# qitianwu/SGFormer

Measured on NVIDIA H100. Metric: nodes/sec fwd+bwd, higher is better.
Workload: dtype bf16

## Files before the change

### include/sgformer_b200.h

```cpp
#ifndef SGFORMER_B200_H
#define SGFORMER_B200_H

#include <stddef.h>
#include <stdint.h>

#ifdef __cplusplus
extern "C" {
#endif

#define SGF_F32 0
#define SGF_BF16 1

#define SGF_ERR_ARG (-1)
#define SGF_ERR_UNSUPPORTED (-2)
#define SGF_ERR_DRIVER (-3)

const char* sgf_version(void);
int64_t sgf_launch_count(void);
int sgf_set_device(int device);

int sgf_csr_build_ws_bytes(int64_t nnz, int64_t n, size_t* bytes );
int sgf_csr_build(const int64_t* edge_index , int64_t nnz, int64_t n, int by_source,
                  int self_loop_mode, int64_t* rowptr , int32_t* col, float* dinv ,
                  void* ws, size_t ws_bytes, void* stream);
// ... 94 lines not shown
    int64_t rows; int32_t n_out;
    int32_t epi;
    void* out; int64_t ldo; int32_t out_dtype;
    const float* bias;
    const void* aux; int64_t ld_aux; int32_t aux_dtype;
    const float* row_scale;
    float alpha, beta;
    const float* alpha_dev; const float* beta_dev;
    int32_t relu, accumulate;
    float nf;
    const float* nf_dev;
    float* den_out;
    const float* r1_row; const float* r1_col;
    float* col_sum; float* col_sumsq;
    int32_t schedule;
} sgf_gemm_nt_args;
int sgf_gemm_nt(const sgf_gemm_nt_args* args , void* stream);

#define SGF_TN_MAX_PAIRS 6
typedef struct {
    const void* a; int64_t lda; int32_t m;
    const void* b; int64_t ldb; int32_t n;
    int64_t rows;
    float* out; int64_t ldo; int32_t transpose_out;
    float alpha, beta; const float* alpha_dev;
    void* ws; size_t ws_bytes;
    int32_t n_pairs;
    int32_t a_off[SGF_TN_MAX_PAIRS], b_off[SGF_TN_MAX_PAIRS];
} sgf_gemm_tn_args;
int sgf_gemm_tn_ws_bytes(int32_t m, int32_t n, int64_t rows, size_t* bytes);
int sgf_gemm_tn(const sgf_gemm_tn_args* args , void* stream);

// ... 135 lines not shown
```

### sgformer_b200/_lib.py

```python
import ctypes as C
import os

from . import _build

_i32, _i64, _f32, _u64, _vp, _sz = C.c_int32, C.c_int64, C.c_float, C.c_uint64, C.c_void_p, C.c_size_t
SGF_MAX_SRC, SGF_MAX_SEG = 4, 16
F32, BF16 = 0, 1
EPI_AFFINE, EPI_ATTN_APPLY, EPI_ATTN_GRAM = 0, 1, 2


class GemmNtArgs(C.Structure):
    _fields_ = [
        ("a", _vp * SGF_MAX_SRC), ("lda", _i64 * SGF_MAX_SRC), ("a_cols", _i64 * SGF_MAX_SRC),
        ("b", _vp * SGF_MAX_SRC), ("ldb", _i64 * SGF_MAX_SRC), ("b_cols", _i64 * SGF_MAX_SRC),
        ("n_a", _i32), ("n_b", _i32), ("n_seg", _i32),
        ("seg_a", _i32 * SGF_MAX_SEG), ("seg_akoff", _i32 * SGF_MAX_SEG), ("seg_b", _i32 * SGF_MAX_SEG),
        ("seg_bkoff", _i32 * SGF_MAX_SEG), ("seg_klen", _i32 * SGF_MAX_SEG),
        ("b_tail", _vp), ("ldb_tail", _i64),
        ("rows", _i64), ("n_out", _i32),
        ("epi", _i32),
        ("out", _vp), ("ldo", _i64), ("out_dtype", _i32),
        ("bias", _vp),
        ("aux", _vp), ("ld_aux", _i64), ("aux_dtype", _i32),
        ("row_scale", _vp),
        ("alpha", _f32), ("beta", _f32),
        ("alpha_dev", _vp), ("beta_dev", _vp),
        ("relu", _i32), ("accumulate", _i32),
        ("nf", _f32), ("nf_dev", _vp),
        ("den_out", _vp),
        ("r1_row", _vp), ("r1_col", _vp),
        ("col_sum", _vp), ("col_sumsq", _vp),
        ("schedule", _i32),
    ]


class AttnGramArgs(C.Structure):
    _fields_ = [
        ("h", _i32), ("m", _i32), ("d", _i32), ("n_nodes", _i64),
        ("wq", _vp), ("bq", _vp), ("wk", _vp), ("bk", _vp), ("wv", _vp), ("bv", _vp),
        ("ld_wq", _i64), ("ld_wk", _i64), ("ld_wv", _i64),
        ("G", _vp), ("s", _vp),
        ("kx", _vp), ("qx", _vp), ("vx", _vp), ("z1", _vp), ("q1", _vp), ("v1", _vp), ("S", _vp),
        ("Bt", _vp), ("tail", _vp), ("bt", _vp), ("sc", _vp),
        ("P", _vp), ("pg", _vp), ("cs", _vp), ("sg", _vp),
        ("dwq", _vp), ("dbq", _vp), ("dwk", _vp), ("dbk", _vp), ("dwv", _vp), ("dbv", _vp),
        ("bcat", _vp), ("a4", _vp),
        ("ws", _vp), ("ws_floats", _i64),
# ... 43 lines not shown
    "sgf_remove_self_loops": (C.c_int, [_vp, _i64, _vp, _vp, _vp, _sz, _vp]),
    "sgf_add_self_loops": (C.c_int, [_vp, _i64, _i64, _vp, _vp]),
    "sgf_subgraph": (C.c_int, [_vp, _i64, _i64, _vp, _i64, _vp, _vp, _vp, _vp, _sz, _vp]),
    "sgf_spmm": (C.c_int, [_vp, _vp, _vp, _vp, _i64, _vp, _i64, _i64, C.c_int, C.c_int, _i64, _vp]),
    "sgf_spmm_flagged": (C.c_int, [_vp, _vp, _vp, _vp, _i64, _vp, _i64, _i64, C.c_int, C.c_int, _i64, _vp, _i64, C.c_int, _vp]),
    "sgf_spmm_range": (C.c_int, [_vp, _vp, _vp, _vp, _i64, _vp, _i64, _i64, C.c_int, C.c_int, _vp, _vp, _vp, _vp, _i64, _vp]),
    "sgf_csr_row_splits": (C.c_int, [_vp, _vp, _i64, _vp, C.c_int, _vp, _vp]),
    "sgf_signal": (C.c_int, [_vp, C.c_uint32, _vp]),
    "sgf_set_dropout_epoch": (C.c_int, [_vp]),
    "sgf_advance_dropout_epoch": (C.c_int, [_vp, _vp]),
    "sgf_memcpy_async": (C.c_int, [_vp, _vp, _sz, _vp]),
    "sgf_wait_flags": (C.c_int, [_vp, C.c_int, _vp]),
    "sgf_csr_build_rot": (C.c_int, [_vp, _i64, _i64, _i64, _i64, C.c_int, C.c_int, _i64, _i64, _vp, _vp, _vp, _vp, _sz, _vp]),
    "sgf_spmm_heavy": (C.c_int, [_vp, _vp, _vp, _i64, _vp, _i64, C.c_int, C.c_int, _vp, _vp, _i64, _vp, _vp, _vp, _i64, _vp]),
    "sgf_gemm_nt": (C.c_int, [C.POINTER(GemmNtArgs), _vp]),
    "sgf_gemm_tn_ws_bytes": (C.c_int, [_i32, _i32, _i64, C.POINTER(_sz)]),
    "sgf_gemm_tn": (C.c_int, [C.POINTER(GemmTnArgs), _vp]),
    "sgf_reduce_ws_bytes": (C.c_int, [_i32, C.POINTER(_sz)]),
    "sgf_colstats": (C.c_int, [_vp, _i64, _i64, C.c_int, C.c_int, _vp, _vp, _vp, _vp, _sz, _vp]),
    "sgf_ln_fwd": (C.c_int, [_vp, _vp, _i64, _i64, C.c_int, C.c_int, _f32, _f32, _vp, _vp, C.c_int, C.c_int, _f32,
                             _u64, _vp, _vp, _vp]),
    "sgf_ln_bwd": (C.c_int, [_vp, _vp, _vp, _i64, _i64, C.c_int, C.c_int, _f32, _f32, _vp, _vp, _vp, C.c_int, C.c_int,
                             _f32, _u64, _f32, _vp, _vp, _vp, _vp, _vp, _sz, _vp]),
    "sgf_ln_bwd_attn": (C.c_int, [_vp, _vp, _vp, _vp, _i64, _i64, C.c_int, C.c_int, _f32, _f32, _vp, _vp, _vp, C.c_int, C.c_int,
                                  _f32, _u64, _f32, _vp, _vp, _vp, _vp, _vp, _vp, _vp, _vp, _vp, _vp, _sz, _vp]),
    "sgf_ln_fwd_graph": (C.c_int, [_vp, _vp, _vp, _i64, _i64, C.c_int, C.c_int, _f32, _f32, _f32, _vp, _vp, C.c_int, C.c_int,
                                   _f32, _u64, _vp, _vp, _vp]),
    "sgf_ln_bwd_attn_graph": (C.c_int, [_vp, _vp, _vp, _vp, _vp, _i64, _i64, C.c_int, C.c_int, _f32, _f32, _f32, _vp, _vp, _vp,
                                        C.c_int, _f32, _u64, _f32, _vp, _vp, _vp, _vp, _vp, _vp, _vp, _vp, _vp, _vp, _vp, _vp,
                                        _sz, _vp]),
# ... 89 lines not shown
```

### sgformer_b200/csrc/gemm_tc.cu

```cuda
#include "common.cuh"
#include "launch_count.h"
#include "../../include/sgformer_b200.h"

#include <cstdlib>
#include <cstring>
#include <mutex>

namespace sgf {

typedef CUresult (*PFN_encodeTiled)(CUtensorMap*, CUtensorMapDataType, cuuint32_t, void*, const cuuint64_t*, const cuuint64_t*,
                                    const cuuint32_t*, const cuuint32_t*, CUtensorMapInterleave, CUtensorMapSwizzle,
                                    CUtensorMapL2promotion, CUtensorMapFloatOOBfill);
static PFN_encodeTiled get_encode() {
    static PFN_encodeTiled fn = nullptr;
    static std::once_flag once;
    std::call_once(once, [] {
        void* p = nullptr;
        cudaDriverEntryPointQueryResult q;
        if (cudaGetDriverEntryPoint("cuTensorMapEncodeTiled", &p, cudaEnableDefault, &q) == cudaSuccess &&
            q == cudaDriverEntryPointSuccess)
            fn = (PFN_encodeTiled)p;
    });
    return fn;
}
// ... 14 lines not shown
    return r == CUDA_SUCCESS ? SGF_OK : SGF_ERR_DRIVER;
}
static int make_tmap_bf16(CUtensorMap* tm, const void* base, int64_t rows, int64_t cols, int64_t ld, int box_rows) {
    return make_tmap_2d(tm, base, 1, rows, cols, ld, box_rows);
}

namespace nt {
constexpr int BM = 128, BK = 64, STAGES = 3;
constexpr int MMA_WARPS = 8;
constexpr int THREADS = 32 * (MMA_WARPS + 4);
constexpr int A_BYTES = BM * BK * 2;
constexpr int B_BYTES_MAX = (256 + 16) * BK * 2;
constexpr int STAGE_BYTES = A_BYTES + B_BYTES_MAX;
constexpr int WSTG_BYTES = 16 * 128;
constexpr int BAR_BYTES = 512;
constexpr int STAT_COLS = 1024;
constexpr int STAT_BYTES = 2 * STAT_COLS * 4;
constexpr int SMEM_BYTES = STAGES * STAGE_BYTES + MMA_WARPS * 2 * WSTG_BYTES + BAR_BYTES + STAT_BYTES + 1024;
constexpr int RES_BYTES = (256 + 16) * 256 * 2;
constexpr int RES_MAX_KB = 16;
constexpr int RES_MIN_STAGES = 3, RING_MAX = 8;
constexpr int SMEM_LIMIT = 232448;
constexpr int RES_FIXED_BYTES = MMA_WARPS * WSTG_BYTES + BAR_BYTES + STAT_BYTES + 1024;
constexpr int SMEM_BYTES_RES = RES_BYTES + RES_MIN_STAGES * A_BYTES + RES_FIXED_BYTES;
static_assert(SMEM_BYTES <= SMEM_LIMIT && SMEM_BYTES_RES <= SMEM_LIMIT, "exceeds the 227 KB of dynamic shared memory per CTA");

struct Seg {
    int a_idx, a_koff, b_idx, b_koff, k_blocks;
};
struct Params {
    int64_t rows;
    int n_out, bn_main, bn_pad, has_tail, n_blocks;
    int64_t num_tiles;
    int b_res;
    int res_bytes, ring_stages;
    int64_t chunk;
    int n_seg, total_kb;
    Seg seg[SGF_MAX_SEG];
    int epi;
    void* out; int64_t ldo; int out_dtype;
    const float* bias;
    const void* aux; int64_t ld_aux; int aux_dtype;
    const float* row_scale;
    float alpha, beta;
    const float* alpha_dev; const float* beta_dev;
    int relu, accumulate;
    float nf; const float* nf_dev; float* den_out;
    const float* r1_row; const float* r1_col;
    int tma_store;
    float* col_sum; float* col_sumsq;
};
struct Tmaps {
    CUtensorMap a[SGF_MAX_SRC];
    CUtensorMap b[SGF_MAX_SRC];
    CUtensorMap tail;
    CUtensorMap out;
};

__device__ __forceinline__ float load1(const void* base, int dtype, int64_t off) {
    return dtype == 1 ? __bfloat162float(static_cast<const __nv_bfloat16*>(base)[off]) : static_cast<const float*>(base)[off];
}
__device__ __forceinline__ void store1(void* base, int dtype, int64_t off, float v) {
    if (dtype == 1) static_cast<__nv_bfloat16*>(base)[off] = __float2bfloat16_rn(v);
    else static_cast<float*>(base)[off] = v;
}
// ... 34 lines not shown
                    c0 += p.chunk;
                    if (c0 >= cnt) return false;
                }
                i = c0;
            }
        }
        const int64_t cend = c0 + p.chunk < cnt ? c0 + p.chunk : cnt;
        m_blk = (int)(blockIdx.x + i * gridDim.x);
        n_blk = nb;
        first = i == c0;
        last = i == cend - 1;
        return true;
    }
};

enum : int { F_BIAS = 1, F_AUX = 2, F_RELU = 4, F_ROWSCALE = 8, F_ACCUM = 16, F_R1 = 32, F_ATTN = 64, F_GENERIC = 128 };

template <bool GEN>
__device__ __forceinline__ void load_piece(const void* src, int dtype, int64_t ld, const int64_t* rows, const bool* row_ok,
                                           int col0, int n_out, bool nc, float* d) {
#pragma unroll
    for (int c = 0; c < 4; ++c)
#pragma unroll
        for (int s = 0; s < 2; ++s) {
            const int col = col0 + 8 * c;
            const int64_t off = rows[s] * ld + col;
            float a0 = 0.f, a1 = 0.f;
            if (!GEN) {
                if (row_ok[s]) {
                    const uint32_t* q = reinterpret_cast<const uint32_t*>(static_cast<const __nv_bfloat16*>(src) + off);
                    unpack_bf16x2(nc ? __ldg(q) : *q, a0, a1);
// ... 2 lines not shown
                if (row_ok[s] && col < n_out) a0 = load1(src, dtype, off);
                if (row_ok[s] && col + 1 < n_out) a1 = load1(src, dtype, off + 1);
            }
            d[4 * c + 2 * s] = a0;
            d[4 * c + 2 * s + 1] = a1;
        }
}

template <int F>
__global__ void __launch_bounds__(THREADS, 1) gemm_nt_kernel(const __grid_constant__ Tmaps tm, const __grid_constant__ Params p) {
    extern __shared__ uint8_t smem_raw[];
    uint8_t* smem = reinterpret_cast<uint8_t*>((reinterpret_cast<uintptr_t>(smem_raw) + 1023) & ~static_cast<uintptr_t>(1023));
    const bool res = p.b_res != 0;
    uint8_t* bres = smem;
    uint8_t* ring = res ? smem + p.res_bytes : smem;
    const int ring_stages = res ? p.ring_stages : STAGES;
    const int ring_stride = res ? A_BYTES : STAGE_BYTES;
    const int stg_per_warp = res ? 1 : 2;
    uint8_t* staging = ring + ring_stages * ring_stride;
    uint64_t* full = reinterpret_cast<uint64_t*>(staging + MMA_WARPS * stg_per_warp * WSTG_BYTES);
    uint64_t* empty = full + RING_MAX;
    uint64_t* bres_full = empty + RING_MAX;
    uint64_t* bres_empty = bres_full + RES_MAX_KB;
    float* stat_sm = reinterpret_cast<float*>(reinterpret_cast<uint8_t*>(full) + BAR_BYTES);
    static_assert((2 * RING_MAX + 2 * RES_MAX_KB) * 8 <= BAR_BYTES, "barrier area");
    static_assert(STAGES <= RING_MAX, "ring barriers");
    const bool want_stats = p.col_sum != nullptr || p.col_sumsq != nullptr;

    const int warp = threadIdx.x >> 5;
    const int lane = threadIdx.x & 31;
    const uint32_t b_tx = p.bn_pad * BK * 2 + (p.has_tail ? 16 * BK * 2 : 0);
    if (want_stats)
        for (int i = threadIdx.x; i < 2 * STAT_COLS; i += THREADS) stat_sm[i] = 0.f;

    if (threadIdx.x == 0) {
        for (int i = 0; i < p.n_seg; ++i) {
            tma_prefetch_desc(&tm.a[p.seg[i].a_idx]);
            tma_prefetch_desc(&tm.b[p.seg[i].b_idx]);
        }
        if (p.has_tail) tma_prefetch_desc(&tm.tail);
        if (p.tma_store) tma_prefetch_desc(&tm.out);
        for (int s = 0; s < ring_stages; ++s) { mbar_init(&full[s], 1); mbar_init(&empty[s], MMA_WARPS); }
        for (int s = 0; s < RES_MAX_KB; ++s) { mbar_init(&bres_full[s], 1); mbar_init(&bres_empty[s], MMA_WARPS); }
        fence_barrier_init();
    }
    __syncthreads();

    if (warp >= MMA_WARPS) {
// ... 31 lines not shown
            }
        }
        return;
    }
    consumer_regs();

    constexpr bool GEN = (F & F_GENERIC) != 0;
    const bool f_bias = GEN ? p.bias != nullptr : (F & F_BIAS) != 0;
    const bool f_aux = GEN ? p.aux != nullptr : (F & F_AUX) != 0;
    const bool f_relu = GEN ? p.relu != 0 : (F & F_RELU) != 0;
    const bool f_rs = GEN ? p.row_scale != nullptr : (F & F_ROWSCALE) != 0;
    const bool f_acc = GEN ? p.accumulate != 0 : (F & F_ACCUM) != 0;
    const bool f_r1 = GEN ? p.r1_row != nullptr : (F & F_R1) != 0;
    const bool f_attn = GEN ? (p.epi == SGF_EPI_ATTN_APPLY || p.epi == SGF_EPI_ATTN_GRAM) : (F & F_ATTN) != 0;
    const bool f_tma = GEN ? p.tma_store != 0 : true;
    const bool f_stats = GEN ? want_stats : false;
    const int out_dtype = GEN ? p.out_dtype : 1;
    const int wg = warp >> 2;
    const int wq = warp & 3;
    const int rr = lane >> 2;
    const int cq = 2 * (lane & 3);
    float alpha = p.alpha, beta = p.beta;
    if (p.alpha_dev) alpha *= *p.alpha_dev;
    if (p.beta_dev) beta *= *p.beta_dev;
    const float nfv = (f_attn && p.nf_dev) ? *p.nf_dev : p.nf;
    const int GW = out_dtype == 1 ? 64 : 32;
    const int ppg = GW / 32;
    const int n_pieces = (p.bn_main + 31) / 32;
    const int nch = p.bn_pad / 64;
    uint8_t* wstg = staging + warp * stg_per_warp * WSTG_BYTES;
    const uint32_t a_off = wg * 64 * BK * 2;

    float acc[4][32];
    float acct[8];
    uint32_t gcount = 0;
    int stage = 0; uint32_t phase = 0;
    TileIter ti(p);
    while (ti.next()) {
        const int m_blk = ti.m_blk, n_blk = ti.n_blk;
        const int64_t row_w = (int64_t)m_blk * BM + wg * 64 + wq * 16;
        const int col_base = n_blk * p.bn_main;
        if (!GEN && (f_acc || f_aux) && lane < 16 && row_w + lane < p.rows) {
            if (f_acc) bulk_prefetch_l2(static_cast<const __nv_bfloat16*>(p.out) + (row_w + lane) * p.ldo + col_base, p.bn_main * 2);
            if (f_aux) bulk_prefetch_l2(static_cast<const __nv_bfloat16*>(p.aux) + (row_w + lane) * p.ld_aux + col_base, p.bn_main * 2);
        }
        int prev = 0;
        for (int kbg = 0; kbg < p.total_kb; ++kbg) {
            if (res && ti.first) mbar_wait(&bres_full[kbg], (uint32_t)(ti.group & 1));
            mbar_wait(&full[stage], phase);
            const uint32_t sa = smem_u32(ring + stage * ring_stride) + a_off;
            const uint32_t sb = res ? smem_u32(bres) + (uint32_t)kbg * b_tx : smem_u32(ring + stage * ring_stride) + A_BYTES;
            wgmma_fence();
#pragma unroll
            for (int k = 0; k < BK / 16; ++k) {
                const uint64_t da = make_smem_desc_sw128(sa + k * 32, 16, 1024);
                const uint32_t sc = (kbg > 0 || k > 0) ? 1u : 0u;
#pragma unroll
                for (int j = 0; j < 4; ++j)
                    if (j < nch) wgmma_n64<0, 0>(acc[j], da, make_smem_desc_sw128(sb + j * 8192 + k * 32, 16, 1024), sc);
                if (p.has_tail) wgmma_n16<0, 0>(acct, da, make_smem_desc_sw128(sb + p.bn_pad * BK * 2 + k * 32, 16, 1024), sc);
            }
            wgmma_commit();
            if (res) wgmma_wait<1>();
            else wgmma_wait<0>();
            __syncwarp();
            if (lane == 0 && (kbg > 0 || !res)) {
                mbar_arrive(&empty[res ? prev : stage]);
                if (res && ti.last) mbar_arrive(&bres_empty[kbg - 1]);
            }
            prev = stage;
            if (++stage == ring_stages) { stage = 0; phase ^= 1; }
        }
        wgmma_wait<0>();
#pragma unroll
        for (int j = 0; j < 4; ++j) fence_regs(acc[j]);
        fence_regs(acct);
        __syncwarp();
        if (lane == 0 && res) {
            mbar_arrive(&empty[prev]);
            if (ti.last) mbar_arrive(&bres_empty[p.total_kb - 1]);
        }

        const int64_t rows[2] = {row_w + rr, row_w + rr + 8};
        const bool row_ok[2] = {rows[0] < p.rows, rows[1] < p.rows};
        float rs[2] = {1.f, 1.f}, r1r[2] = {0.f, 0.f}, inv_den[2] = {1.f, 1.f};
#pragma unroll
        for (int s = 0; s < 2; ++s) {
            if (f_rs && row_ok[s]) rs[s] = p.row_scale[rows[s]];
            if (f_r1 && row_ok[s]) r1r[s] = p.r1_row[rows[s]];
        }
        if (f_attn) {
#pragma unroll
            for (int s = 0; s < 2; ++s) {
                const float den = __shfl_sync(0xffffffffu, acct[2 * s], lane & ~3) + nfv;
                inv_den[s] = 1.f / den;
                if (row_ok[s] && p.den_out && n_blk == 0 && (lane & 3) == 0) p.den_out[rows[s]] = den;
// ... 9 lines not shown
                    if (stg_per_warp == 2) bulk_wait_read<1>(); else bulk_wait_read<0>();
                }
                __syncwarp();
            }
            float v[16];
#pragma unroll
            for (int i = 0; i < 16; ++i) v[i] = acc[pc >> 1][(pc & 1) * 16 + i];
            const int col0 = col_base + pc * 32 + cq;
            float ax[16], old[16];
            if (f_aux) load_piece<GEN>(p.aux, p.aux_dtype, p.ld_aux, rows, row_ok, col0, p.n_out, true, ax);
            if (f_acc) load_piece<GEN>(p.out, out_dtype, p.ldo, rows, row_ok, col0, p.n_out, false, old);
#pragma unroll
            for (int i = 0; i < 16; ++i) {
                const int s = (i >> 1) & 1;
                const int col = col0 + 8 * (i >> 2) + (i & 1);
                const bool cok = !GEN || col < p.n_out;
                float x = v[i];
                if (f_attn) {
                    if (f_aux) x += nfv * ax[i];
                    if (f_bias && cok) x += __ldg(p.bias + col);
                    x *= inv_den[s];
                } else {
                    x *= alpha;
                    if (f_aux) x += beta * ax[i];
                    if (f_bias && cok) x += __ldg(p.bias + col);
                    if (f_r1 && cok) x += r1r[s] * __ldg(p.r1_col + col);
                    if (f_relu) x = fmaxf(x, 0.f);
                    if (f_rs) x *= rs[s];
                }
                if (f_acc) x += old[i];
                v[i] = x;
// ... 12 lines not shown
                            const int chunk = (2 * c + (cq >> 2)) ^ (r & 7);
                            *reinterpret_cast<float2*>(tile + r * 128 + chunk * 16 + 4 * (cq & 3)) = make_float2(v[4 * c + 2 * s], v[4 * c + 2 * s + 1]);
                        }
                    }
            } else if constexpr (GEN) {
#pragma unroll
                for (int i = 0; i < 16; ++i) {
                    const int s = (i >> 1) & 1;
                    const int col = col0 + 8 * (i >> 2) + (i & 1);
                    if (row_ok[s] && col < p.n_out) store1(p.out, out_dtype, rows[s] * p.ldo + col, v[i]);
                }
            }
            if (f_tma && (pp == ppg - 1 || pc == n_pieces - 1)) {
                fence_proxy_async_smem();
                __syncwarp();
                if (lane == 0) {
                    tma_store_2d(&tm.out, wstg + buf * WSTG_BYTES, col_base + g * GW, (int32_t)row_w);
                    bulk_commit();
                }
                if (f_stats) {
                    const uint8_t* tile = wstg + buf * WSTG_BYTES;
                    const int64_t valid_rows = p.rows - row_w;
                    for (int cg = lane; cg < GW; cg += 32) {
                        const int colg = col_base + g * GW + cg;
                        if (colg >= p.n_out || colg >= col_base + p.bn_main) continue;
                        float s1 = 0.f, s2 = 0.f;
                        for (int r = 0; r < 16 && r < valid_rows; ++r) {
                            float x;
                            if (out_dtype == 1) {
                                const int chunk = (cg >> 3) ^ (r & 7);
                                x = __bfloat162float(*reinterpret_cast<const __nv_bfloat16*>(tile + r * 128 + chunk * 16 + (cg & 7) * 2));
                            } else {
                                const int chunk = (cg >> 2) ^ (r & 7);
                                x = *reinterpret_cast<const float*>(tile + r * 128 + chunk * 16 + (cg & 3) * 4);
                            }
                            s1 += x;
                            s2 += x * x;
                        }
                        atomicAdd(&stat_sm[colg], s1);
                        atomicAdd(&stat_sm[STAT_COLS + colg], s2);
                    }
                }
                ++gcount;
            }
        }
    }
    if (f_tma && lane == 0) bulk_wait<0>();
    if (f_stats) {
        named_bar_sync(3, 32 * MMA_WARPS);
        for (int i = threadIdx.x; i < p.n_out; i += 32 * MMA_WARPS) {
            if (p.col_sum) atomicAdd(&p.col_sum[i], stat_sm[i]);
            if (p.col_sumsq) atomicAdd(&p.col_sumsq[i], stat_sm[STAT_COLS + i]);
        }
    }
}
}

constexpr int FLUSH_KB = 16;
#ifndef SGF_TN_DIAG
#define SGF_TN_DIAG 0
#endif

__device__ __forceinline__ void red_add_f32(float* p, float v) {
    asm volatile("red.global.add.f32 [%0], %1;" :: "l"(p), "f"(v) : "memory");
}
__device__ __forceinline__ void flush_acc_red(float (&acc)[4][32], float* ws, int mp, int mrow, int cq, int j0, int ncols, bool add) {
#pragma unroll
    for (int j = 0; j < 4; ++j) {
// ... 303 lines not shown
        } else {
            i = t - h * h;
            c = un;
        }
        float acc = 0.f;
        for (int part = 0; part < nparts; ++part) acc += ws[((int64_t)part * (un + 1) + c) * mp + i];
        if (t < h * h) G[(int64_t)(t / h) * ldg + t % h] = acc;
        else s[i] = acc;
    }
}
}
}

using namespace sgf;

extern "C" int sgf_gemm_nt(const sgf_gemm_nt_args* a, void* stream) {
    if (!a || a->rows < 0 || a->n_out <= 0 || a->n_seg <= 0 || a->n_seg > SGF_MAX_SEG || a->n_a <= 0 || a->n_a > SGF_MAX_SRC ||
        a->n_b <= 0 || a->n_b > SGF_MAX_SRC || !a->out)
        return SGF_ERR_ARG;
    if (a->out_dtype != 0 && a->out_dtype != 1) return SGF_ERR_ARG;
    if (a->aux && a->aux_dtype != 0 && a->aux_dtype != 1) return SGF_ERR_ARG;
    if (a->rows == 0) return SGF_OK;
    const bool has_tail = a->b_tail != nullptr;
    if (has_tail && (a->n_b != 1 || a->n_out > 256)) return SGF_ERR_ARG;
    if (a->epi == SGF_EPI_ATTN_APPLY && (!has_tail || !a->aux)) return SGF_ERR_ARG;
    if (a->epi == SGF_EPI_ATTN_GRAM && (!has_tail || !a->bias || !a->nf_dev || a->aux)) return SGF_ERR_ARG;
    if (a->epi != SGF_EPI_AFFINE && a->epi != SGF_EPI_ATTN_APPLY && a->epi != SGF_EPI_ATTN_GRAM) return SGF_ERR_ARG;
    if ((a->r1_row == nullptr) != (a->r1_col == nullptr)) return SGF_ERR_ARG;

    nt::Params p;
// ... 47 lines not shown
    if (has_tail && (rc = make_tmap_bf16(&tm.tail, a->b_tail, 16, a->b_cols[0], a->ldb_tail, 16))) return rc;

    p.epi = a->epi;
    p.out = a->out; p.ldo = a->ldo; p.out_dtype = a->out_dtype;
    p.bias = a->bias;
    p.aux = a->aux; p.ld_aux = a->ld_aux; p.aux_dtype = a->aux_dtype;
    p.row_scale = a->row_scale;
    p.alpha = a->alpha; p.beta = a->beta; p.alpha_dev = a->alpha_dev; p.beta_dev = a->beta_dev;
    p.relu = a->relu; p.accumulate = a->accumulate;
    p.nf = a->nf; p.nf_dev = a->nf_dev; p.den_out = a->den_out;
    p.r1_row = a->r1_row; p.r1_col = a->r1_col;
    {
        const int es = a->out_dtype == 1 ? 2 : 4;
        p.tma_store = ((reinterpret_cast<uintptr_t>(a->out) & 15) == 0 && (a->ldo * es) % 16 == 0) ? 1 : 0;
        if (p.tma_store && (rc = make_tmap_2d(&tm.out, a->out, a->out_dtype, a->rows, a->n_out, a->ldo, 16))) return rc;
        p.col_sum = a->col_sum; p.col_sumsq = a->col_sumsq;
        if ((p.col_sum || p.col_sumsq) && (!p.tma_store || a->n_out > nt::STAT_COLS)) return SGF_ERR_UNSUPPORTED;
    }

    {
        const int64_t b_tx = (int64_t)(p.bn_pad + (has_tail ? 16 : 0)) * nt::BK * 2;
        const bool fits = p.total_kb <= nt::RES_MAX_KB && b_tx * p.total_kb <= nt::RES_BYTES;
        if (a->schedule == SGF_GEMM_RESIDENT_B && !fits) return SGF_ERR_UNSUPPORTED;
        p.b_res = (fits && (a->schedule == SGF_GEMM_RESIDENT_B || (a->schedule == SGF_GEMM_AUTO && p.n_blocks == 1))) ? 1 : 0;
        p.chunk = p.n_blocks == 1 ? (int64_t)1 << 40 : 4;
        p.res_bytes = (int)(b_tx * p.total_kb);
        const int st = (nt::SMEM_LIMIT - p.res_bytes - nt::RES_FIXED_BYTES) / nt::A_BYTES;
        p.ring_stages = st < nt::RING_MAX ? st : nt::RING_MAX;
        if (p.b_res && p.ring_stages < nt::RES_MIN_STAGES) return SGF_ERR_UNSUPPORTED;
    }
    const int64_t work = p.b_res ? m_blocks : p.num_tiles;
    const int64_t grid = work < num_sms() ? work : num_sms();
    const int smem_bytes = p.b_res ? p.res_bytes + p.ring_stages * nt::A_BYTES + nt::RES_FIXED_BYTES : nt::SMEM_BYTES;

    int feat = (a->bias ? nt::F_BIAS : 0) | (a->aux ? nt::F_AUX : 0) | (a->relu ? nt::F_RELU : 0) |
               (a->row_scale ? nt::F_ROWSCALE : 0) | (a->accumulate ? nt::F_ACCUM : 0) | (a->r1_row ? nt::F_R1 : 0) |
               (a->epi != SGF_EPI_AFFINE ? nt::F_ATTN : 0);
    const bool al16 = (!a->bias || (reinterpret_cast<uintptr_t>(a->bias) & 15) == 0) &&
                      (!a->r1_col || (reinterpret_cast<uintptr_t>(a->r1_col) & 15) == 0) &&
                      (!a->aux || (a->aux_dtype == 1 && (reinterpret_cast<uintptr_t>(a->aux) & 15) == 0 && (a->ld_aux * 2) % 16 == 0));
    const bool fast_ok = p.tma_store && a->out_dtype == 1 && a->n_out % 32 == 0 && al16 && !p.col_sum && !p.col_sumsq &&
                         p.n_blocks * p.bn_main == a->n_out;
    static const bool no_special = [] { const char* e = getenv("SGF_GEMM_NT_GENERIC"); return e && e[0] == '1'; }();
    if (!fast_ok || no_special) feat = nt::F_GENERIC;
    const int smem_max = nt::SMEM_LIMIT;
#define SGF_NT_CASE(FEAT)                                                                                                   \
    case (FEAT): {                                                                                                         \
        static bool attr_set = false;                                                                                      \
        if (!attr_set) {                                                                                                   \
            SGF_CUDA_TRY(cudaFuncSetAttribute(nt::gemm_nt_kernel<(FEAT)>, cudaFuncAttributeMaxDynamicSharedMemorySize,     \
                                              smem_max));                                                                  \
            attr_set = true;                                                                                               \
        }                                                                                                                  \
        nt::gemm_nt_kernel<(FEAT)><<<(unsigned)grid, nt::THREADS, smem_bytes, (cudaStream_t)stream>>>(tm, p);              \
        launched = true;                                                                                                   \
    } break;
    for (int attempt = 0; attempt < 2; ++attempt) {
        bool launched = false;
        switch (feat) {
            SGF_NT_CASE(0)
            SGF_NT_CASE(nt::F_BIAS)
            SGF_NT_CASE(nt::F_BIAS | nt::F_RELU)
            SGF_NT_CASE(nt::F_ROWSCALE)
            SGF_NT_CASE(nt::F_ACCUM)
            SGF_NT_CASE(nt::F_AUX)
            SGF_NT_CASE(nt::F_AUX | nt::F_ACCUM)
            SGF_NT_CASE(nt::F_AUX | nt::F_BIAS)
            SGF_NT_CASE(nt::F_AUX | nt::F_R1)
            SGF_NT_CASE(nt::F_AUX | nt::F_ATTN)
            SGF_NT_CASE(nt::F_BIAS | nt::F_ATTN)
            SGF_NT_CASE(nt::F_BIAS | nt::F_R1)
            SGF_NT_CASE(nt::F_BIAS | nt::F_R1 | nt::F_ACCUM)
            SGF_NT_CASE(nt::F_GENERIC)
            default: break;
        }
        if (launched) break;
        feat = nt::F_GENERIC;
    }
#undef SGF_NT_CASE
    SGF_LAUNCH_CHECK(); count_launch();
    return SGF_OK;
}

static inline int tn_splits(int64_t kb_total, int m_blocks) {
    const int64_t cap = num_sms() / m_blocks > 0 ? num_sms() / m_blocks : 1;
    return (int)(kb_total < cap ? (kb_total < 1 ? 1 : kb_total) : cap);
}

extern "C" int sgf_gemm_tn_ws_bytes(int32_t m, int32_t n, int64_t rows, size_t* bytes) {
    if (!bytes || m <= 0 || m > 256 || n <= 0 || n > 256 || rows < 0) return SGF_ERR_ARG;
    const int m_blocks = (m + 127) / 128, un = (n + 15) / 16 * 16;
// ... 126 lines not shown
```

### sgformer_b200/kernels.py

```python
from __future__ import annotations

import ctypes as C
import os
import threading
from dataclasses import dataclass
from typing import Optional, Sequence, Tuple

import torch

from . import _lib
from ._lib import BF16, EPI_AFFINE, EPI_ATTN_APPLY, EPI_ATTN_GRAM, F32, AttnGramArgs, GemmNtArgs, GemmTnArgs, check

Tensor = torch.Tensor
_tls = threading.local()


def lib():
    return _lib.load()


def _use(t: Tensor):
    if not t.is_cuda:
        raise RuntimeError("sgformer_b200 kernels need CUDA tensors (no CPU fallback); got device " + str(t.device))
    idx = t.device.index if t.device.index is not None else torch.cuda.current_device()
# ... 588 lines not shown
        raise ValueError(f"out is {tuple(out.shape)}, expected ({rows}, {n_out})")
    args.out, args.ldo, args.out_dtype = out.data_ptr(), ldo, dcode(out)
    args.bias = _p(_f32vec(bias, n_out, "bias"))
    if aux is not None:
        ar, ac, lda_ = _mat(aux, "aux")
        if ar != rows or ac != n_out:
            raise ValueError("aux shape mismatch")
        args.aux, args.ld_aux, args.aux_dtype = aux.data_ptr(), lda_, dcode(aux)
    args.row_scale = _p(_f32vec(row_scale, rows, "row_scale"))
    args.alpha, args.beta = alpha, beta
    args.alpha_dev, args.beta_dev = _p(alpha_dev), _p(beta_dev)
    args.relu, args.accumulate = int(relu), int(accumulate)
    args.nf, args.den_out = nf, _p(_f32vec(den_out, rows, "den_out"))
    args.nf_dev = _p(_f32vec(nf_dev, 1, "nf_dev"))
    args.r1_row, args.r1_col = _p(_f32vec(r1_row, rows, "r1_row")), _p(_f32vec(r1_col, n_out, "r1_col"))
    fused_stats = (col_sum is not None or col_sumsq is not None) and stats_fusable(out)
    if fused_stats:
        args.col_sum, args.col_sumsq = _p(_f32vec(col_sum, n_out, "col_sum")), _p(_f32vec(col_sumsq, n_out, "col_sumsq"))
    args.schedule = GEMM_NT_SCHEDULE if schedule is None else schedule
    check(lib().sgf_gemm_nt(C.byref(args), _stream()), "sgf_gemm_nt")
    if (col_sum is not None or col_sumsq is not None) and not fused_stats:
        s_, q_ = colstats(out, want_sum=col_sum is not None, want_sumsq=col_sumsq is not None)
        if col_sum is not None:
            col_sum.add_(s_)
        if col_sumsq is not None:
            col_sumsq.add_(q_)
    return out


GEMM_NT_SCHEDULE = int(os.environ.get("SGF_GEMM_NT_SCHEDULE", "0"))

FUSE_GEMM_STATS = os.environ.get("SGF_FUSED_STATS", "0") == "1"


def stats_fusable(out: Tensor) -> bool:
    return FUSE_GEMM_STATS and out.data_ptr() % 16 == 0 and (out.stride(0) * out.element_size()) % 16 == 0 and \
        out.shape[1] <= 1024


def _tn_once(a: Tensor, lda: int, m: int, b: Tensor, ldb: int, n: int, rows: int, out: Tensor, transpose_out: bool,
             alpha: float, beta: float, alpha_dev: Optional[Tensor], pairs: Sequence[Tuple[int, int]] = ()):
    nbytes = C.c_size_t(0)
    check(lib().sgf_gemm_tn_ws_bytes(m, n, rows, C.byref(nbytes)), "sgf_gemm_tn_ws_bytes")
    ws = torch.empty(max(nbytes.value, 4), dtype=torch.uint8, device=out.device)
    args = GemmTnArgs()
    args.a, args.lda, args.m = a.data_ptr(), lda, m
    args.b, args.ldb, args.n = b.data_ptr(), ldb, n
    args.rows = rows
    args.out, args.ldo, args.transpose_out = out.data_ptr(), out.stride(0), int(transpose_out)
    args.alpha, args.beta, args.alpha_dev = alpha, beta, _p(alpha_dev)
    args.ws, args.ws_bytes = ws.data_ptr(), nbytes.value
    args.n_pairs = len(pairs)
# ... 537 lines not shown
```

Baseline: 12.65 million.

## Add specialized fused column-stats and f32-output paths to NT GEMM with dynamic ring stages

Column sum and sum-of-squares now accumulate in registers per warp and are reduced once per CTA into a global partial buffer, with the last CTA (found via an atomic counter) doing the final cross-CTA reduction. This replaces the old shared-memory atomics in the generic path, which also frees the fixed stats shared-memory region. A specialized f32-output template is added, and the streaming ring's stage count is now sized from the actual B tile size, so smaller tiles get deeper pipelines. Fused stats remain off by default behind SGF_FUSED_STATS and need a workspace allocation plus a memset per call.

New measurement: 12.70 million (median of 6 runs). No clear change (+0.4%).

```diff
diff --git a/include/sgformer_b200.h b/include/sgformer_b200.h
--- a/include/sgformer_b200.h
+++ b/include/sgformer_b200.h
@@ -132,8 +132,10 @@
     const float* r1_row; const float* r1_col;
     float* col_sum; float* col_sumsq;
     int32_t schedule;
+    void* stat_ws; size_t stat_ws_bytes;
 } sgf_gemm_nt_args;
 int sgf_gemm_nt(const sgf_gemm_nt_args* args , void* stream);
+int sgf_gemm_nt_stats_ws_bytes(int32_t n_out, size_t* bytes);
 
 #define SGF_TN_MAX_PAIRS 6
 typedef struct {
diff --git a/sgformer_b200/_lib.py b/sgformer_b200/_lib.py
--- a/sgformer_b200/_lib.py
+++ b/sgformer_b200/_lib.py
@@ -5,6 +5,7 @@
 
 _i32, _i64, _f32, _u64, _vp, _sz = C.c_int32, C.c_int64, C.c_float, C.c_uint64, C.c_void_p, C.c_size_t
 SGF_MAX_SRC, SGF_MAX_SEG = 4, 16
+SGF_ERR_UNSUPPORTED = -2
 F32, BF16 = 0, 1
 EPI_AFFINE, EPI_ATTN_APPLY, EPI_ATTN_GRAM = 0, 1, 2
 
@@ -31,6 +32,7 @@
         ("r1_row", _vp), ("r1_col", _vp),
         ("col_sum", _vp), ("col_sumsq", _vp),
         ("schedule", _i32),
+        ("stat_ws", _vp), ("stat_ws_bytes", _sz),
     ]
 
 
@@ -104,6 +106,7 @@
     "sgf_csr_build_rot": (C.c_int, [_vp, _i64, _i64, _i64, _i64, C.c_int, C.c_int, _i64, _i64, _vp, _vp, _vp, _vp, _sz, _vp]),
     "sgf_spmm_heavy": (C.c_int, [_vp, _vp, _vp, _i64, _vp, _i64, C.c_int, C.c_int, _vp, _vp, _i64, _vp, _vp, _vp, _i64, _vp]),
     "sgf_gemm_nt": (C.c_int, [C.POINTER(GemmNtArgs), _vp]),
+    "sgf_gemm_nt_stats_ws_bytes": (C.c_int, [_i32, C.POINTER(_sz)]),
     "sgf_gemm_tn_ws_bytes": (C.c_int, [_i32, _i32, _i64, C.POINTER(_sz)]),
     "sgf_gemm_tn": (C.c_int, [C.POINTER(GemmTnArgs), _vp]),
     "sgf_reduce_ws_bytes": (C.c_int, [_i32, C.POINTER(_sz)]),
diff --git a/sgformer_b200/csrc/gemm_tc.cu b/sgformer_b200/csrc/gemm_tc.cu
--- a/sgformer_b200/csrc/gemm_tc.cu
+++ b/sgformer_b200/csrc/gemm_tc.cu
@@ -52,14 +52,14 @@
 constexpr int STAGE_BYTES = A_BYTES + B_BYTES_MAX;
 constexpr int WSTG_BYTES = 16 * 128;
 constexpr int BAR_BYTES = 512;
-constexpr int STAT_COLS = 1024;
-constexpr int STAT_BYTES = 2 * STAT_COLS * 4;
-constexpr int SMEM_BYTES = STAGES * STAGE_BYTES + MMA_WARPS * 2 * WSTG_BYTES + BAR_BYTES + STAT_BYTES + 1024;
+constexpr int STAT_COLS = 256;
+constexpr int STREAM_FIXED_BYTES = MMA_WARPS * 2 * WSTG_BYTES + BAR_BYTES + 1024;
+constexpr int SMEM_BYTES = STAGES * STAGE_BYTES + STREAM_FIXED_BYTES;
 constexpr int RES_BYTES = (256 + 16) * 256 * 2;
 constexpr int RES_MAX_KB = 16;
 constexpr int RES_MIN_STAGES = 3, RING_MAX = 8;
 constexpr int SMEM_LIMIT = 232448;
-constexpr int RES_FIXED_BYTES = MMA_WARPS * WSTG_BYTES + BAR_BYTES + STAT_BYTES + 1024;
+constexpr int RES_FIXED_BYTES = MMA_WARPS * WSTG_BYTES + BAR_BYTES + 1024;
 constexpr int SMEM_BYTES_RES = RES_BYTES + RES_MIN_STAGES * A_BYTES + RES_FIXED_BYTES;
 static_assert(SMEM_BYTES <= SMEM_LIMIT && SMEM_BYTES_RES <= SMEM_LIMIT, "exceeds the 227 KB of dynamic shared memory per CTA");
 
@@ -72,6 +72,7 @@
     int64_t num_tiles;
     int b_res;
     int res_bytes, ring_stages;
+    int stage_bytes;
     int64_t chunk;
     int n_seg, total_kb;
     Seg seg[SGF_MAX_SEG];
@@ -87,6 +88,7 @@
     const float* r1_row; const float* r1_col;
     int tma_store;
     float* col_sum; float* col_sumsq;
+    float* stat_part; unsigned* stat_cnt;
 };
 struct Tmaps {
     CUtensorMap a[SGF_MAX_SRC];
@@ -151,7 +153,67 @@
     }
 };
 
-enum : int { F_BIAS = 1, F_AUX = 2, F_RELU = 4, F_ROWSCALE = 8, F_ACCUM = 16, F_R1 = 32, F_ATTN = 64, F_GENERIC = 128 };
+enum : int { F_BIAS = 1, F_AUX = 2, F_RELU = 4, F_ROWSCALE = 8, F_ACCUM = 16, F_R1 = 32, F_ATTN = 64, F_GENERIC = 128,
+             F_F32 = 256, F_STATS = 512 };
+
+#ifndef SGF_NT_DIAG
+#define SGF_NT_DIAG 0
+#endif
+
+__device__ __forceinline__ void stats_flush(const Params& p, const float (&s1)[4][2], const float (&s2)[4][2], uint8_t* staging,
+                                            int stg_stride, float* grp_sm, unsigned* last_sm, int warp, int lane) {
+    const int n = p.n_out;
+    float* mine = reinterpret_cast<float*>(staging + warp * stg_stride);
+#pragma unroll
+    for (int g = 0; g < 4; ++g) {
+        const int c = 64 * g + 2 * lane;
+        if (c < n) {
+            *reinterpret_cast<float2*>(mine + c) = make_float2(s1[g][0], s1[g][1]);
+            *reinterpret_cast<float2*>(mine + STAT_COLS + c) = make_float2(s2[g][0], s2[g][1]);
+        }
+    }
+    named_bar_sync(3, 32 * MMA_WARPS);
+    float* part = p.stat_part + (size_t)blockIdx.x * 2 * n;
+    for (int i = threadIdx.x; i < 2 * n; i += 32 * MMA_WARPS) {
+        const int off = i < n ? i : STAT_COLS + i - n;
+        float t = 0.f;
+        for (int w = 0; w < MMA_WARPS; ++w) t += reinterpret_cast<const float*>(staging + w * stg_stride)[off];
+        part[i] = t;
+    }
+    __threadfence();
+    named_bar_sync(3, 32 * MMA_WARPS);
+    if (threadIdx.x == 0) *last_sm = atomicAdd(p.stat_cnt, 1u) == gridDim.x - 1;
+    named_bar_sync(3, 32 * MMA_WARPS);
+    if (!*last_sm) return;
+    __threadfence();
+    const int nv = 2 * n / 4, G = 32 * MMA_WARPS / nv, grp = threadIdx.x / nv, v = threadIdx.x % nv;
+    if (grp < G) {
+        float4 a[4];
+#pragma unroll
+        for (int j = 0; j < 4; ++j) a[j] = make_float4(0.f, 0.f, 0.f, 0.f);
+        unsigned b = grp;
+        for (; b + 3 * G < gridDim.x; b += 4 * G)
+#pragma unroll
+            for (int j = 0; j < 4; ++j) {
+                const float4 x = __ldcg(reinterpret_cast<const float4*>(p.stat_part + (size_t)(b + j * G) * 2 * n) + v);
+                a[j].x += x.x; a[j].y += x.y; a[j].z += x.z; a[j].w += x.w;
+            }
+        for (; b < gridDim.x; b += G) {
+            const float4 x = __ldcg(reinterpret_cast<const float4*>(p.stat_part + (size_t)b * 2 * n) + v);
+            a[0].x += x.x; a[0].y += x.y; a[0].z += x.z; a[0].w += x.w;
+        }
+        reinterpret_cast<float4*>(grp_sm)[grp * nv + v] =
+            make_float4((a[0].x + a[1].x) + (a[2].x + a[3].x), (a[0].y + a[1].y) + (a[2].y + a[3].y),
+                        (a[0].z + a[1].z) + (a[2].z + a[3].z), (a[0].w + a[1].w) + (a[2].w + a[3].w));
+    }
+    named_bar_sync(3, 32 * MMA_WARPS);
+    for (int i = threadIdx.x; i < 2 * n; i += 32 * MMA_WARPS) {
+        float t = 0.f;
+        for (int q = 0; q < G; ++q) t += grp_sm[q * 2 * n + i];
+        float* dst = i < n ? p.col_sum + i : p.col_sumsq + (i - n);
+        if (i < n ? p.col_sum != nullptr : p.col_sumsq != nullptr) *dst += t;
+    }
+}
 
 template <bool GEN>
 __device__ __forceinline__ void load_piece(const void* src, int dtype, int64_t ld, const int64_t* rows, const bool* row_ok,
@@ -184,24 +246,22 @@
     const bool res = p.b_res != 0;
     uint8_t* bres = smem;
     uint8_t* ring = res ? smem + p.res_bytes : smem;
-    const int ring_stages = res ? p.ring_stages : STAGES;
-    const int ring_stride = res ? A_BYTES : STAGE_BYTES;
+    const int ring_stages = p.ring_stages;
+    const int ring_stride = res ? A_BYTES : p.stage_bytes;
     const int stg_per_warp = res ? 1 : 2;
     uint8_t* staging = ring + ring_stages * ring_stride;
     uint64_t* full = reinterpret_cast<uint64_t*>(staging + MMA_WARPS * stg_per_warp * WSTG_BYTES);
     uint64_t* empty = full + RING_MAX;
     uint64_t* bres_full = empty + RING_MAX;
     uint64_t* bres_empty = bres_full + RES_MAX_KB;
-    float* stat_sm = reinterpret_cast<float*>(reinterpret_cast<uint8_t*>(full) + BAR_BYTES);
-    static_assert((2 * RING_MAX + 2 * RES_MAX_KB) * 8 <= BAR_BYTES, "barrier area");
+    unsigned* last_sm = reinterpret_cast<unsigned*>(bres_empty + RES_MAX_KB);
+    float* grp_sm = reinterpret_cast<float*>(ring);
+    static_assert((2 * RING_MAX + 2 * RES_MAX_KB) * 8 + 4 <= BAR_BYTES, "barrier area");
     static_assert(STAGES <= RING_MAX, "ring barriers");
-    const bool want_stats = p.col_sum != nullptr || p.col_sumsq != nullptr;
 
     const int warp = threadIdx.x >> 5;
     const int lane = threadIdx.x & 31;
     const uint32_t b_tx = p.bn_pad * BK * 2 + (p.has_tail ? 16 * BK * 2 : 0);
-    if (want_stats)
-        for (int i = threadIdx.x; i < 2 * STAT_COLS; i += THREADS) stat_sm[i] = 0.f;
 
     if (threadIdx.x == 0) {
         for (int i = 0; i < p.n_seg; ++i) {
@@ -263,8 +323,9 @@
     const bool f_r1 = GEN ? p.r1_row != nullptr : (F & F_R1) != 0;
     const bool f_attn = GEN ? (p.epi == SGF_EPI_ATTN_APPLY || p.epi == SGF_EPI_ATTN_GRAM) : (F & F_ATTN) != 0;
     const bool f_tma = GEN ? p.tma_store != 0 : true;
-    const bool f_stats = GEN ? want_stats : false;
-    const int out_dtype = GEN ? p.out_dtype : 1;
+    constexpr bool f_stats = (F & F_STATS) != 0;
+    constexpr bool RAGGED = GEN || (F & F_F32) != 0;
+    const int out_dtype = GEN ? p.out_dtype : ((F & F_F32) ? 0 : 1);
     const int wg = warp >> 2;
     const int wq = warp & 3;
     const int rr = lane >> 2;
@@ -282,6 +343,9 @@
 
     float acc[4][32];
     float acct[8];
+    float st1[4][2], st2[4][2];
+#pragma unroll
+    for (int g = 0; g < 4; ++g) st1[g][0] = st1[g][1] = st2[g][0] = st2[g][1] = 0.f;
     uint32_t gcount = 0;
     int stage = 0; uint32_t phase = 0;
     TileIter ti(p);
@@ -302,6 +366,7 @@
             wgmma_fence();
 #pragma unroll
             for (int k = 0; k < BK / 16; ++k) {
+                if (SGF_NT_DIAG == 2) break;
                 const uint64_t da = make_smem_desc_sw128(sa + k * 32, 16, 1024);
                 const uint32_t sc = (kbg > 0 || k > 0) ? 1u : 0u;
 #pragma unroll
@@ -329,6 +394,7 @@
             mbar_arrive(&empty[prev]);
             if (ti.last) mbar_arrive(&bres_empty[p.total_kb - 1]);
         }
+        if (SGF_NT_DIAG == 1) continue;
 
         const int64_t rows[2] = {row_w + rr, row_w + rr + 8};
         const bool row_ok[2] = {rows[0] < p.rows, rows[1] < p.rows};
@@ -368,7 +434,7 @@
             for (int i = 0; i < 16; ++i) {
                 const int s = (i >> 1) & 1;
                 const int col = col0 + 8 * (i >> 2) + (i & 1);
-                const bool cok = !GEN || col < p.n_out;
+                const bool cok = !RAGGED || col < p.n_out;
                 float x = v[i];
                 if (f_attn) {
                     if (f_aux) x += nfv * ax[i];
@@ -411,31 +477,22 @@
             if (f_tma && (pp == ppg - 1 || pc == n_pieces - 1)) {
                 fence_proxy_async_smem();
                 __syncwarp();
-                if (lane == 0) {
+                if (lane == 0 && SGF_NT_DIAG != 3) {
                     tma_store_2d(&tm.out, wstg + buf * WSTG_BYTES, col_base + g * GW, (int32_t)row_w);
                     bulk_commit();
                 }
                 if (f_stats) {
                     const uint8_t* tile = wstg + buf * WSTG_BYTES;
                     const int64_t valid_rows = p.rows - row_w;
-                    for (int cg = lane; cg < GW; cg += 32) {
-                        const int colg = col_base + g * GW + cg;
-                        if (colg >= p.n_out || colg >= col_base + p.bn_main) continue;
-                        float s1 = 0.f, s2 = 0.f;
+                    if (g * GW + 2 * lane < p.bn_main) {
                         for (int r = 0; r < 16 && r < valid_rows; ++r) {
-                            float x;
-                            if (out_dtype == 1) {
-                                const int chunk = (cg >> 3) ^ (r & 7);
-                                x = __bfloat162float(*reinterpret_cast<const __nv_bfloat16*>(tile + r * 128 + chunk * 16 + (cg & 7) * 2));
-                            } else {
-                                const int chunk = (cg >> 2) ^ (r & 7);
-                                x = *reinterpret_cast<const float*>(tile + r * 128 + chunk * 16 + (cg & 3) * 4);
-                            }
-                            s1 += x;
-                            s2 += x * x;
+                            float x0, x1;
+                            unpack_bf16x2(*reinterpret_cast<const uint32_t*>(tile + r * 128 + (((lane >> 2) ^ (r & 7)) * 16) + (lane & 3) * 4), x0, x1);
+                            st1[g][0] += x0;
+                            st1[g][1] += x1;
+                            st2[g][0] = fmaf(x0, x0, st2[g][0]);
+                            st2[g][1] = fmaf(x1, x1, st2[g][1]);
                         }
-                        atomicAdd(&stat_sm[colg], s1);
-                        atomicAdd(&stat_sm[STAT_COLS + colg], s2);
                     }
                 }
                 ++gcount;
@@ -443,12 +500,9 @@
         }
     }
     if (f_tma && lane == 0) bulk_wait<0>();
-    if (f_stats) {
-        named_bar_sync(3, 32 * MMA_WARPS);
-        for (int i = threadIdx.x; i < p.n_out; i += 32 * MMA_WARPS) {
-            if (p.col_sum) atomicAdd(&p.col_sum[i], stat_sm[i]);
-            if (p.col_sumsq) atomicAdd(&p.col_sumsq[i], stat_sm[STAT_COLS + i]);
-        }
+    if constexpr (f_stats) {
+        __syncwarp();
+        stats_flush(p, st1, st2, staging, stg_per_warp * WSTG_BYTES, grp_sm, last_sm, warp, lane);
     }
 }
 }
@@ -782,6 +836,12 @@
 
 using namespace sgf;
 
+extern "C" int sgf_gemm_nt_stats_ws_bytes(int32_t n_out, size_t* bytes) {
+    if (!bytes || n_out <= 0) return SGF_ERR_ARG;
+    *bytes = 256 + (size_t)num_sms() * 2 * (size_t)n_out * sizeof(float);
+    return SGF_OK;
+}
+
 extern "C" int sgf_gemm_nt(const sgf_gemm_nt_args* a, void* stream) {
     if (!a || a->rows < 0 || a->n_out <= 0 || a->n_seg <= 0 || a->n_seg > SGF_MAX_SEG || a->n_a <= 0 || a->n_a > SGF_MAX_SRC ||
         a->n_b <= 0 || a->n_b > SGF_MAX_SRC || !a->out)
@@ -859,8 +919,6 @@
         const int es = a->out_dtype == 1 ? 2 : 4;
         p.tma_store = ((reinterpret_cast<uintptr_t>(a->out) & 15) == 0 && (a->ldo * es) % 16 == 0) ? 1 : 0;
         if (p.tma_store && (rc = make_tmap_2d(&tm.out, a->out, a->out_dtype, a->rows, a->n_out, a->ldo, 16))) return rc;
-        p.col_sum = a->col_sum; p.col_sumsq = a->col_sumsq;
-        if ((p.col_sum || p.col_sumsq) && (!p.tma_store || a->n_out > nt::STAT_COLS)) return SGF_ERR_UNSUPPORTED;
     }
 
     {
@@ -873,10 +931,16 @@
         const int st = (nt::SMEM_LIMIT - p.res_bytes - nt::RES_FIXED_BYTES) / nt::A_BYTES;
         p.ring_stages = st < nt::RING_MAX ? st : nt::RING_MAX;
         if (p.b_res && p.ring_stages < nt::RES_MIN_STAGES) return SGF_ERR_UNSUPPORTED;
+        if (!p.b_res) {
+            p.stage_bytes = (int)(nt::A_BYTES + b_tx);
+            const int ss = (nt::SMEM_LIMIT - nt::STREAM_FIXED_BYTES) / p.stage_bytes;
+            p.ring_stages = ss < nt::RING_MAX ? ss : nt::RING_MAX;
+        }
     }
     const int64_t work = p.b_res ? m_blocks : p.num_tiles;
     const int64_t grid = work < num_sms() ? work : num_sms();
-    const int smem_bytes = p.b_res ? p.res_bytes + p.ring_stages * nt::A_BYTES + nt::RES_FIXED_BYTES : nt::SMEM_BYTES;
+    const int smem_bytes = p.b_res ? p.res_bytes + p.ring_stages * nt::A_BYTES + nt::RES_FIXED_BYTES
+                                   : p.ring_stages * p.stage_bytes + nt::STREAM_FIXED_BYTES;
 
     int feat = (a->bias ? nt::F_BIAS : 0) | (a->aux ? nt::F_AUX : 0) | (a->relu ? nt::F_RELU : 0) |
                (a->row_scale ? nt::F_ROWSCALE : 0) | (a->accumulate ? nt::F_ACCUM : 0) | (a->r1_row ? nt::F_R1 : 0) |
@@ -884,10 +948,23 @@
     const bool al16 = (!a->bias || (reinterpret_cast<uintptr_t>(a->bias) & 15) == 0) &&
                       (!a->r1_col || (reinterpret_cast<uintptr_t>(a->r1_col) & 15) == 0) &&
                       (!a->aux || (a->aux_dtype == 1 && (reinterpret_cast<uintptr_t>(a->aux) & 15) == 0 && (a->ld_aux * 2) % 16 == 0));
-    const bool fast_ok = p.tma_store && a->out_dtype == 1 && a->n_out % 32 == 0 && al16 && !p.col_sum && !p.col_sumsq &&
+    const bool fast_ok = p.tma_store && a->out_dtype == 1 && a->n_out % 32 == 0 && al16 &&
                          p.n_blocks * p.bn_main == a->n_out;
+    const bool f32_ok = p.tma_store && a->out_dtype == 0 && p.n_blocks == 1 && al16;
     static const bool no_special = [] { const char* e = getenv("SGF_GEMM_NT_GENERIC"); return e && e[0] == '1'; }();
-    if (!fast_ok || no_special) feat = nt::F_GENERIC;
+    if (f32_ok && !no_special) feat |= nt::F_F32;
+    else if (!fast_ok || no_special) feat = nt::F_GENERIC;
+    if (a->col_sum || a->col_sumsq) {
+        if (feat & (nt::F_GENERIC | nt::F_F32) || p.n_blocks != 1 || a->n_out > nt::STAT_COLS) return SGF_ERR_UNSUPPORTED;
+        size_t need = 0;
+        sgf_gemm_nt_stats_ws_bytes(a->n_out, &need);
+        if (!a->stat_ws || a->stat_ws_bytes < need || (reinterpret_cast<uintptr_t>(a->stat_ws) & 15)) return SGF_ERR_ARG;
+        feat |= nt::F_STATS;
+        p.col_sum = a->col_sum; p.col_sumsq = a->col_sumsq;
+        p.stat_cnt = static_cast<unsigned*>(a->stat_ws);
+        p.stat_part = reinterpret_cast<float*>(static_cast<uint8_t*>(a->stat_ws) + 256);
+        SGF_CUDA_TRY(cudaMemsetAsync(a->stat_ws, 0, sizeof(unsigned), (cudaStream_t)stream));
+    }
     const int smem_max = nt::SMEM_LIMIT;
 #define SGF_NT_CASE(FEAT)                                                                                                   \
     case (FEAT): {                                                                                                         \
@@ -916,10 +993,13 @@
             SGF_NT_CASE(nt::F_BIAS | nt::F_ATTN)
             SGF_NT_CASE(nt::F_BIAS | nt::F_R1)
             SGF_NT_CASE(nt::F_BIAS | nt::F_R1 | nt::F_ACCUM)
+            SGF_NT_CASE(nt::F_BIAS | nt::F_F32)
+            SGF_NT_CASE(nt::F_BIAS | nt::F_STATS)
             SGF_NT_CASE(nt::F_GENERIC)
             default: break;
         }
         if (launched) break;
+        if (feat & nt::F_STATS) return SGF_ERR_UNSUPPORTED;
         feat = nt::F_GENERIC;
     }
 #undef SGF_NT_CASE
diff --git a/sgformer_b200/kernels.py b/sgformer_b200/kernels.py
--- a/sgformer_b200/kernels.py
+++ b/sgformer_b200/kernels.py
@@ -626,12 +626,25 @@
     args.nf, args.den_out = nf, _p(_f32vec(den_out, rows, "den_out"))
     args.nf_dev = _p(_f32vec(nf_dev, 1, "nf_dev"))
     args.r1_row, args.r1_col = _p(_f32vec(r1_row, rows, "r1_row")), _p(_f32vec(r1_col, n_out, "r1_col"))
-    fused_stats = (col_sum is not None or col_sumsq is not None) and stats_fusable(out)
-    if fused_stats:
+    args.schedule = GEMM_NT_SCHEDULE if schedule is None else schedule
+    want_stats = col_sum is not None or col_sumsq is not None
+    fused_stats = False
+    if want_stats and stats_fusable(out):
         args.col_sum, args.col_sumsq = _p(_f32vec(col_sum, n_out, "col_sum")), _p(_f32vec(col_sumsq, n_out, "col_sumsq"))
-    args.schedule = GEMM_NT_SCHEDULE if schedule is None else schedule
-    check(lib().sgf_gemm_nt(C.byref(args), _stream()), "sgf_gemm_nt")
-    if (col_sum is not None or col_sumsq is not None) and not fused_stats:
+        nbytes = C.c_size_t(0)
+        check(lib().sgf_gemm_nt_stats_ws_bytes(n_out, C.byref(nbytes)), "sgf_gemm_nt_stats_ws_bytes")
+        ws = torch.empty(nbytes.value, dtype=torch.uint8, device=out.device)
+        args.stat_ws, args.stat_ws_bytes = ws.data_ptr(), nbytes.value
+        rc = lib().sgf_gemm_nt(C.byref(args), _stream())
+        fused_stats = rc != _lib.SGF_ERR_UNSUPPORTED
+        if fused_stats:
+            check(rc, "sgf_gemm_nt")
+        else:
+            args.col_sum = args.col_sumsq = args.stat_ws = None
+            args.stat_ws_bytes = 0
+    if not fused_stats:
+        check(lib().sgf_gemm_nt(C.byref(args), _stream()), "sgf_gemm_nt")
+    if want_stats and not fused_stats:
         s_, q_ = colstats(out, want_sum=col_sum is not None, want_sumsq=col_sumsq is not None)
         if col_sum is not None:
             col_sum.add_(s_)
@@ -646,8 +659,9 @@
 
 
 def stats_fusable(out: Tensor) -> bool:
-    return FUSE_GEMM_STATS and out.data_ptr() % 16 == 0 and (out.stride(0) * out.element_size()) % 16 == 0 and \
-        out.shape[1] <= 1024
+    n = out.shape[1]
+    return FUSE_GEMM_STATS and out.dtype == torch.bfloat16 and out.data_ptr() % 16 == 0 and \
+        (out.stride(0) * out.element_size()) % 16 == 0 and n % 32 == 0 and n <= 256
 
 
 def _tn_once(a: Tensor, lda: int, m: int, b: Tensor, ldb: int, n: int, rows: int, out: Tensor, transpose_out: bool,
```
